# stone-d-chen/ffvvc

Measured on AMD Instinct MI355X. Metric: decoded frames/sec (4K/8K 10-bit VVC) per GPU, higher is better.
Workload: dtype u16

## Files before the change

### ffvvc_amd/csrc/affine.hip

```cpp
#include "common.hpp"
#include "runtime.hpp"
#include "../../include/vvc_mi355.h"

namespace vvc355 {

#define VVC355_TABLE(type, name, count) __device__ static const type a_tab_##name[count]
#include "tables.inc"
#undef VVC355_TABLE

static constexpr int kAwP = 12;

struct AffineLds {
    uint16_t win[11 * kAwP];
    int16_t th[11 * 4];
    int16_t pp[2][6 * 6];
};

__device__ __forceinline__ void group16_sync()
{
    __builtin_amdgcn_fence(__ATOMIC_ACQ_REL, "wavefront");
    __builtin_amdgcn_wave_barrier();
}

template <int BD>
__global__ __launch_bounds__(256) void affine_kernel(const vvc355_affine_job *__restrict__ jobs, int n_jobs)
{
    using px_t = typename Px<BD>::type;
    __shared__ __attribute__((aligned(16))) AffineLds lds_all[16];
    const int ji = blockIdx.x * 16 + (threadIdx.x >> 4), l = threadIdx.x & 15;
    if (ji >= n_jobs)
        return;
    AffineLds &L = lds_all[threadIdx.x >> 4];
    const vvc355_affine_job job = jobs[ji];
    const int x = l & 3, y = l >> 2;
    const int16_t *dmv = (const int16_t *)job.diff_mv;
    const bool bi = job.pred_flag == 3;
    int val[2] = { 0, 0 };

#pragma unroll
    for (int i = 0; i < 2; i++) {
        if (!(job.pred_flag & (1 << i)))
            continue;
        const int mvx = job.mv[2 * i], mvy = job.mv[2 * i + 1];
        const int mx = mvx & 15, my = mvy & 15;
        const int ox = job.x + (mvx >> 4), oy = job.y + (mvy >> 4);
        const uint8_t *plane = (const uint8_t *)(i ? job.ref1 : job.ref0);
        const int stride = i ? job.ref1_stride : job.ref0_stride;
        const bool prof = i ? job.prof1 : job.prof0;
#pragma unroll
        for (int it = 0; it < 8; it++) {
            const int e = l + 16 * it;
            if (e < 121) {
                const int r = e / 11, c = e - r * 11;
                const int xa = clip3(ox - 3 + c, 0, job.pic_w - 1), ya = clip3(oy - 3 + r, 0, job.pic_h - 1);
                L.win[r * kAwP + c] = (uint16_t)gld<px_t>(plane + (ptrdiff_t)ya * stride + xa * (int)sizeof(px_t));
            }
        }
        group16_sync();
        const int8_t *hf = a_tab_inter_luma_filters + (2 * 16 + mx) * 8, *vf = a_tab_inter_luma_filters + (2 * 16 + my) * 8;
        int p;
        if (mx) {
            const int r0 = my ? 0 : 3, nr = my ? 11 : 4;
            for (int e = l; e < nr * 4; e += 16) {
                const int r = r0 + (e >> 2), c = e & 3;
                int s = 0;
#pragma unroll
                for (int k = 0; k < 8; k++) s += hf[k] * (int)L.win[r * kAwP + c + k];
                L.th[r * 4 + c] = (int16_t)(s >> (BD - 8));
            }
            group16_sync();
            if (my) {
                int s = 0;
#pragma unroll
                for (int k = 0; k < 8; k++) s += vf[k] * (int)L.th[(y + k) * 4 + x];
                p = s >> 6;
            } else {
                p = L.th[(y + 3) * 4 + x];
            }
        } else if (my) {
            int s = 0;
#pragma unroll
            for (int k = 0; k < 8; k++) s += vf[k] * (int)L.win[(y + k) * kAwP + x + 3];
            p = s >> (BD - 8);
        } else {
            p = (int)L.win[(y + 3) * kAwP + x + 3] << (14 - BD);
        }
        p = (int16_t)p;
        if (prof) {
            int16_t *pp = L.pp[i];
            pp[(y + 1) * 6 + x + 1] = (int16_t)p;
            for (int e = l; e < 20; e += 16) {
                int rx, ry;
                if (e < 6)       { ry = -1; rx = e - 1; }
                else if (e < 12) { ry = 4;  rx = e - 7; }
                else             { const int k = e - 12; ry = k >> 1; rx = (k & 1) ? 4 : -1; }
                const int s = L.win[(ry + (my >> 3) + 3) * kAwP + rx + (mx >> 3) + 3];
                pp[(ry + 1) * 6 + rx + 1] = (int16_t)(s << (14 - BD));
            }
            group16_sync();
            const int o = (y + 1) * 6 + x + 1;
            const int g_h = (int16_t)((pp[o + 1] >> 6) - (pp[o - 1] >> 6));
            const int g_v = (int16_t)((pp[o + 6] >> 6) - (pp[o - 6] >> 6));
            const int limit = 1 << max(13, BD + 1);
            const int di = g_h * (int)dmv[i * 32 + l] + g_v * (int)dmv[i * 32 + 16 + l];
            p = p + clip3(di, -limit, limit - 1);
        }
        val[i] = p;
        group16_sync();
        if (!bi) {
            uint8_t *drow = (uint8_t *)job.dst + (ptrdiff_t)y * job.dst_stride;
            int out;
            if (!job.weight_flag) {
                const int sh = 14 - BD;
                out = (p + (1 << (sh - 1))) >> sh;
            } else {
                const int sh = job.denom + (prof ? max(2, 14 - BD) : 14 - BD);
                out = ((p * job.w0 + (1 << (sh - 1))) >> sh) + job.o0 * (1 << (BD - 8));
            }
            st_px<BD>(drow, x, lmcs_fwd<BD>((const uint8_t *)job.lmcs_lut, clip_px<BD>(out)));
        }
    }
    if (bi) {
        const int a = (int16_t)val[0], b = (int16_t)val[1];
        uint8_t *drow = (uint8_t *)job.dst + (ptrdiff_t)y * job.dst_stride;
        int out;
        if (!job.weight_flag) {
            const int sh = max(3, 15 - BD);
            out = (a + b + (1 << (sh - 1))) >> sh;
        } else {
            const int sh = job.denom + max(3, 15 - BD);
            out = (a * job.w0 + b * job.w1 + ((((job.o0 + job.o1) << (BD - 8)) + 1) << (sh - 1))) >> sh;
        }
        st_px<BD>(drow, x, lmcs_fwd<BD>((const uint8_t *)job.lmcs_lut, clip_px<BD>(out)));
    }
}

}

extern "C" void vvc355_affine_batch(void *stream, int bd, const vvc355_affine_job *jobs_dev, int n_jobs)
{
    using namespace vvc355;
    if (n_jobs <= 0) return;
    VVC355_BD_DISPATCH(bd, hipLaunchKernelGGL((affine_kernel<BD>), dim3((n_jobs + 15) / 16), dim3(256), 0, (hipStream_t)stream, jobs_dev, n_jobs));
    HIP_CHECK(hipGetLastError());
}
```

Baseline: 554.0.

## Restructure affine luma MC with packed sdot2 taps, vectorized window loads, prefetch

Rewrites the affine 4x4 inter-prediction kernel. Both reference windows are now fetched up front with vector loads when in bounds, falling back to clipped per-pixel loads only at picture edges. Filter taps are precomputed as packed 16-bit pairs so horizontal and vertical filtering use sdot2, with the copy/h/v special cases removed on the strength of a static assertion that fraction zero is an identity filter. The job descriptor is loaded cooperatively into LDS, PROF deltas are prefetched, and one barrier per list is dropped for uni-prediction. The cost is more registers and LDS per job, and full 8-tap filtering even for integer motion vectors.

After: 553.9. About the same (-0.0%).

```diff
diff --git a/ffvvc_amd/csrc/affine.hip b/ffvvc_amd/csrc/affine.hip
--- a/ffvvc_amd/csrc/affine.hip
+++ b/ffvvc_amd/csrc/affine.hip
@@ -1,20 +1,54 @@
+#include <type_traits>
 #include "common.hpp"
 #include "runtime.hpp"
 #include "../../include/vvc_mi355.h"
 
 namespace vvc355 {
 
-#define VVC355_TABLE(type, name, count) __device__ static const type a_tab_##name[count]
+#define VVC355_TABLE(type, name, count) __device__ static constexpr type a_tab_##name[count]
 #include "tables.inc"
 #undef VVC355_TABLE
 
+struct AffineTaps { uint32_t v[16 * 16]; };
+constexpr uint32_t affine_pack16(int lo, int hi) { return ((uint32_t)lo & 0xffffu) | ((uint32_t)hi & 0xffffu) << 16; }
+constexpr AffineTaps make_affine_taps()
+{
+    AffineTaps t{};
+    for (int f = 0; f < 16; f++) {
+        const int8_t *c = a_tab_inter_luma_filters + (2 * 16 + f) * 8;
+        uint32_t *v = t.v + f * 16;
+        for (int m = 0; m < 4; m++) v[m] = affine_pack16(c[2 * m], c[2 * m + 1]);
+        v[8] = affine_pack16(0, c[0]);
+        for (int m = 1; m < 4; m++) v[8 + m] = affine_pack16(c[2 * m - 1], c[2 * m]);
+        v[12] = affine_pack16(c[7], 0);
+    }
+    return t;
+}
+__device__ static constexpr AffineTaps a_affine_taps __attribute__((aligned(16))) = make_affine_taps();
+constexpr bool affine_zero_fraction_is_identity()
+{
+    for (int k = 0; k < 8; k++)
+        if (a_tab_inter_luma_filters[2 * 16 * 8 + k] != (k == 3 ? 64 : 0))
+            return false;
+    return true;
+}
+static_assert(affine_zero_fraction_is_identity(), "ff_vvc_inter_luma_filters[2][0] must be {0,0,0,64,0,0,0,0}: the kernel has no copy / h / v cases");
+
+typedef short affine_v2s __attribute__((ext_vector_type(2)));
+__device__ __forceinline__ int affine_dot2(uint32_t a, uint32_t b, int acc)
+{
+    return __builtin_amdgcn_sdot2(__builtin_bit_cast(affine_v2s, a), __builtin_bit_cast(affine_v2s, b), acc, false);
+}
+
 static constexpr int kAwP = 12;
 
 struct AffineLds {
-    uint16_t win[11 * kAwP];
-    int16_t th[11 * 4];
+    vvc355_affine_job job;
+    uint16_t win[2][11 * kAwP];
+    int16_t thT[4 * kAwP];
     int16_t pp[2][6 * 6];
 };
+static_assert(sizeof(vvc355_affine_job) == 96 && sizeof(AffineLds) % 16 == 0 && offsetof(AffineLds, win) % 8 == 0, "vector access to the LDS planes");
 
 __device__ __forceinline__ void group16_sync()
 {
@@ -26,66 +60,121 @@
 __global__ __launch_bounds__(256) void affine_kernel(const vvc355_affine_job *__restrict__ jobs, int n_jobs)
 {
     using px_t = typename Px<BD>::type;
+    constexpr int ISZ = (int)sizeof(px_t);
     __shared__ __attribute__((aligned(16))) AffineLds lds_all[16];
     const int ji = blockIdx.x * 16 + (threadIdx.x >> 4), l = threadIdx.x & 15;
     if (ji >= n_jobs)
         return;
     AffineLds &L = lds_all[threadIdx.x >> 4];
-    const vvc355_affine_job job = jobs[ji];
+    if (l < 12)
+        ((uint2 *)&L.job)[l] = gld<uint2>((const uint8_t *)(jobs + ji) + 8 * l);
+    group16_sync();
+    const vvc355_affine_job job = L.job;
     const int x = l & 3, y = l >> 2;
     const int16_t *dmv = (const int16_t *)job.diff_mv;
     const bool bi = job.pred_flag == 3;
     int val[2] = { 0, 0 };
 
+    typename std::conditional<(BD > 8), uint2, uint32_t>::type q[2][3] = {};
+    uint4 he[2] = {}, ho[2] = {}, vt[2] = {};
+    uint32_t ho4[2] = {}, vt4[2] = {};
+    int dmx[2] = { 0, 0 }, dmy[2] = { 0, 0 };
+    bool fast[2] = { false, false };
 #pragma unroll
     for (int i = 0; i < 2; i++) {
         if (!(job.pred_flag & (1 << i)))
             continue;
         const int mvx = job.mv[2 * i], mvy = job.mv[2 * i + 1];
-        const int mx = mvx & 15, my = mvy & 15;
         const int ox = job.x + (mvx >> 4), oy = job.y + (mvy >> 4);
         const uint8_t *plane = (const uint8_t *)(i ? job.ref1 : job.ref0);
         const int stride = i ? job.ref1_stride : job.ref0_stride;
+        fast[i] = ox >= 3 && ox + 9 <= job.pic_w && oy >= 3 && oy + 8 <= job.pic_h;
+        if (fast[i] && (l & 3) < 3) {
+            const uint8_t *org = plane + row_off(oy - 3, stride) + (ox - 3 + 4 * (l & 3)) * ISZ;
+#pragma unroll
+            for (int it = 0; it < 3; it++) {
+                const uint32_t off = (uint32_t)__mul24(min((l >> 2) + 4 * it, 10), stride);
+                if constexpr (BD > 8) q[i][it] = gld<uint2>(org + off);
+                else                  q[i][it] = gld<uint32_t>(org + off);
+            }
+        }
+        const uint32_t *ht = a_affine_taps.v + (mvx & 15) * 16, *vp = a_affine_taps.v + (mvy & 15) * 16 + (y & 1) * 8;
+        he[i] = gld<uint4>(ht);
+        ho[i] = gld<uint4>(ht + 8);
+        ho4[i] = gld<uint32_t>(ht + 12);
+        vt[i] = gld<uint4>(vp);
+        vt4[i] = gld<uint32_t>(vp + 4);
+        if (i ? job.prof1 : job.prof0) {
+            dmx[i] = gld<int16_t>(dmv + i * 32 + l);
+            dmy[i] = gld<int16_t>(dmv + i * 32 + 16 + l);
+        }
+    }
+#pragma unroll
+    for (int i = 0; i < 2; i++) {
+        if (!(job.pred_flag & (1 << i)))
+            continue;
+        if (fast[i]) {
+            if ((l & 3) < 3) {
+#pragma unroll
+                for (int it = 0; it < 3; it++) {
+                    const int r = (l >> 2) + 4 * it;
+                    uint2 v;
+                    if constexpr (BD > 8) v = q[i][it];
+                    else v = make_uint2(__builtin_amdgcn_perm(0, q[i][it], 0x0c010c00u), __builtin_amdgcn_perm(0, q[i][it], 0x0c030c02u));
+                    if (r < 11)
+                        *(uint2 *)&L.win[i][r * kAwP + 4 * (l & 3)] = v;
+                }
+            }
+        } else if (l < kAwP) {
+            const int ox = job.x + (job.mv[2 * i] >> 4), oy = job.y + (job.mv[2 * i + 1] >> 4);
+            const uint8_t *plane = (const uint8_t *)(i ? job.ref1 : job.ref0);
+            const int stride = i ? job.ref1_stride : job.ref0_stride;
+            const int xa = clip3(ox - 3 + l, 0, job.pic_w - 1) * ISZ;
+#pragma unroll
+            for (int r = 0; r < 11; r++) {
+                const int ya = clip3(oy - 3 + r, 0, job.pic_h - 1);
+                L.win[i][r * kAwP + l] = (uint16_t)gld<px_t>(plane + (uint32_t)(__mul24(ya, stride) + xa));
+            }
+        }
+    }
+    group16_sync();
+
+#pragma unroll
+    for (int i = 0; i < 2; i++) {
+        if (!(job.pred_flag & (1 << i)))
+            continue;
+        const int mx = job.mv[2 * i] & 15, my = job.mv[2 * i + 1] & 15;
         const bool prof = i ? job.prof1 : job.prof0;
-#pragma unroll
-        for (int it = 0; it < 8; it++) {
-            const int e = l + 16 * it;
-            if (e < 121) {
-                const int r = e / 11, c = e - r * 11;
-                const int xa = clip3(ox - 3 + c, 0, job.pic_w - 1), ya = clip3(oy - 3 + r, 0, job.pic_h - 1);
-                L.win[r * kAwP + c] = (uint16_t)gld<px_t>(plane + (ptrdiff_t)ya * stride + xa * (int)sizeof(px_t));
+        {
+            const uint32_t e[4] = { he[i].x, he[i].y, he[i].z, he[i].w }, o[5] = { ho[i].x, ho[i].y, ho[i].z, ho[i].w, ho4[i] };
+#pragma unroll
+            for (int trip = 0; trip < 2; trip++) {
+                const int it = l + 16 * trip;
+                if (it < 22) {
+                    const int r = it >> 1, xp = it & 1;
+                    const uint32_t *d = (const uint32_t *)L.win[i] + r * (kAwP / 2) + xp;
+                    int a = 0, b = 0;
+#pragma unroll
+                    for (int m = 0; m < 5; m++) {
+                        const uint32_t s = d[m];
+                        if (m < 4) a = affine_dot2(s, e[m], a);
+                        b = affine_dot2(s, o[m], b);
+                    }
+                    L.thT[(2 * xp) * kAwP + r] = (int16_t)(a >> (BD - 8));
+                    L.thT[(2 * xp + 1) * kAwP + r] = (int16_t)(b >> (BD - 8));
+                }
             }
         }
         group16_sync();
-        const int8_t *hf = a_tab_inter_luma_filters + (2 * 16 + mx) * 8, *vf = a_tab_inter_luma_filters + (2 * 16 + my) * 8;
         int p;
-        if (mx) {
-            const int r0 = my ? 0 : 3, nr = my ? 11 : 4;
-            for (int e = l; e < nr * 4; e += 16) {
-                const int r = r0 + (e >> 2), c = e & 3;
-                int s = 0;
-#pragma unroll
-                for (int k = 0; k < 8; k++) s += hf[k] * (int)L.win[r * kAwP + c + k];
-                L.th[r * 4 + c] = (int16_t)(s >> (BD - 8));
-            }
-            group16_sync();
-            if (my) {
-                int s = 0;
-#pragma unroll
-                for (int k = 0; k < 8; k++) s += vf[k] * (int)L.th[(y + k) * 4 + x];
-                p = s >> 6;
-            } else {
-                p = L.th[(y + 3) * 4 + x];
-            }
-        } else if (my) {
+        {
+            const uint32_t t[5] = { vt[i].x, vt[i].y, vt[i].z, vt[i].w, vt4[i] };
+            const uint32_t *d = (const uint32_t *)L.thT + x * (kAwP / 2) + (y >> 1);
             int s = 0;
 #pragma unroll
-            for (int k = 0; k < 8; k++) s += vf[k] * (int)L.win[(y + k) * kAwP + x + 3];
-            p = s >> (BD - 8);
-        } else {
-            p = (int)L.win[(y + 3) * kAwP + x + 3] << (14 - BD);
-        }
-        p = (int16_t)p;
+            for (int m = 0; m < 5; m++) s = affine_dot2(d[m], t[m], s);
+            p = (int16_t)(s >> 6);
+        }
         if (prof) {
             int16_t *pp = L.pp[i];
             pp[(y + 1) * 6 + x + 1] = (int16_t)p;
@@ -94,7 +183,7 @@
                 if (e < 6)       { ry = -1; rx = e - 1; }
                 else if (e < 12) { ry = 4;  rx = e - 7; }
                 else             { const int k = e - 12; ry = k >> 1; rx = (k & 1) ? 4 : -1; }
-                const int s = L.win[(ry + (my >> 3) + 3) * kAwP + rx + (mx >> 3) + 3];
+                const int s = L.win[i][(ry + (my >> 3) + 3) * kAwP + rx + (mx >> 3) + 3];
                 pp[(ry + 1) * 6 + rx + 1] = (int16_t)(s << (14 - BD));
             }
             group16_sync();
@@ -102,11 +191,12 @@
             const int g_h = (int16_t)((pp[o + 1] >> 6) - (pp[o - 1] >> 6));
             const int g_v = (int16_t)((pp[o + 6] >> 6) - (pp[o - 6] >> 6));
             const int limit = 1 << max(13, BD + 1);
-            const int di = g_h * (int)dmv[i * 32 + l] + g_v * (int)dmv[i * 32 + 16 + l];
+            const int di = g_h * dmx[i] + g_v * dmy[i];
             p = p + clip3(di, -limit, limit - 1);
         }
         val[i] = p;
-        group16_sync();
+        if (bi)
+            group16_sync();
         if (!bi) {
             uint8_t *drow = (uint8_t *)job.dst + (ptrdiff_t)y * job.dst_stride;
             int out;
```
